# John-Ragland/pygenray

Hardware: AMD Instinct MI355X
Metric: ray-steps/sec (whole node), 1e5-ray Munk fan to 1000 km; eigenray wall-clock (higher is better)
Workload: dtype f64

## Files before the change

pygenray_amd/csrc/pgr_device.h:

```cpp
#ifndef PGR_DEVICE_H
#define PGR_DEVICE_H

struct EnvDev {
    const double2* tab;
    const double* rin;
    const double* zin;
    const double* depths;
    const double* depth_ranges;
    const double* pp;
    int nr, nz, nb;
    int row_stride;
    int z_uniform, r_uniform, b_uniform;
    int beta_zero;
    int z_pow2;
    int z_simple;
    double b_zmin, b_xlo, b_xhi;
    double z0, dz, inv_dz;
    double r0, dr, inv_dr;
    double b0, db, inv_db;
    double zlo_tol, zhi_tol, rlo_tol, rhi_tol;
    double c_lo, c_hi;
    const unsigned short* zbucket;
    int z_bucket, zb_B;
    double zb_z0, zb_inv_w;
// ... 49 lines not shown
              "kFanArgsKernargOffset together with the kernel's signature");

#define RUNNING (-1)


__device__ __forceinline__ double frcp(double b)
{
    double y = __builtin_amdgcn_rcp(b);
    double e = fma(-b, y, 1.0);
    y = fma(y, e, y);
    e = fma(-b, y, 1.0);
    y = fma(y, e, y);
    return y;
}
__device__ __forceinline__ double fdiv(double a, double b)
{
    double y = __builtin_amdgcn_rcp(b);
    double e = fma(-b, y, 1.0);
    y = fma(y, e, y);
    double q = a * y;
    double r = fma(-q, b, a);
    return fma(r, y, q);
}
__device__ __forceinline__ double frcp_seed(double b)
{
    double y = __builtin_amdgcn_rcp(b);
    double e = fma(-b, y, 1.0);
    return fma(y, e, y);
}
__device__ __forceinline__ double fdiv_y(double a, double b, double y)
{
    double q = a * y;
    double r = fma(-q, b, a);
    return fma(r, y, q);
}
__device__ __forceinline__ double frsqrt_raw(double x)
{
    double y = __builtin_amdgcn_rsq(x);
    double e = fma(-x * y, y, 1.0);
    y = fma(y * 0.5, e, y);
    e = fma(-x * y, y, 1.0);
    y = fma(y * 0.5, e, y);
    return y;
}
__device__ __forceinline__ double fsqrt(double x)
{
    double y = __builtin_amdgcn_rsq(x);
    double e = fma(-x * y, y, 1.0);
    y = fma(y * 0.5, e, y);
    double g = x * y;
    double d = fma(-g, g, x);
    double r = fma(d * 0.5, y, g);
    return (x == 0.0 || x == INFINITY) ? x : r;
}
__device__ __forceinline__ double frsqrt(double x)
{
#ifdef PGR_FMA
    return frsqrt_raw(x);
#else
    double y = __builtin_amdgcn_rsq(x);
    double e = fma(-x * y, y, 1.0);
    y = fma(y * 0.5, e, y);
    double g = x * y;
    double d = fma(-g, g, x);
    double s = fma(d * 0.5, y, g);
    y = __longlong_as_double(__double_as_longlong(y) | 1LL);
    double r = fma(-s, y, 1.0);
    double out = fma(y, r, y);
    return out;
#endif
}
__device__ __forceinline__ double pow_m02(double x, const double fifth = 0.2, const double kln2 = PGR_CR_POW_KLN2)
{
    return pgr_cr_pow_m02_k(x, fifth, kln2);
}
__device__ __forceinline__ double min_step_of(double t)
{
    long long b = __double_as_longlong(t);
    double nx = (t == 0.0) ? 4.9406564584124654e-324 : __longlong_as_double(t > 0 ? b + 1 : b - 1);
    return 10 * fabs(nx - t);
}
__device__ __forceinline__ double grid_at(double g0, double dg, int j)
{
#pragma clang fp contract(off)
    double m = (double)j * dg;
    return g0 + m;
}

__device__ __forceinline__ unsigned long long ballot64(bool b) { return __builtin_amdgcn_ballot_w64(b); }

__device__ __forceinline__ int clamp_index(int j, int hi)
{
    int r;
    asm("v_med3_i32 %0, %1, 0, %2" : "=v"(r) : "v"(j), "s"(hi));
    return r;
}

__device__ __forceinline__ int cell_uniform(double q, double g0, double dg, double inv_dg, int n)
{
    double t = (q - g0) * inv_dg;
    t = fmin(fmax(t, -1.0), (double)n);
    int j = (int)floor(t);
    double gj = grid_at(g0, dg, j), gj1 = grid_at(g0, dg, j + 1);
    j += (gj >= q) ? -1 : ((gj1 < q) ? 1 : 0);
    return min(max(j, 0), n - 2);
}

__device__ __forceinline__ int cell_search(double q, const double* __restrict__ g, int n)
{
    int lo = 0, hi = n;
    while (lo < hi) {
        int mid = (lo + hi) >> 1;
        if (g[mid] < q) lo = mid + 1; else hi = mid;
    }
    return min(max(lo - 1, 0), n - 2);
}

#define A21 (1.0 / 5)
#define A31 (3.0 / 40)
#define A32 (9.0 / 40)
#define A41 (44.0 / 45)
#define A42 (-56.0 / 15)
#define A43 (32.0 / 9)
#define A51 (19372.0 / 6561)
#define A52 (-25360.0 / 2187)
#define A53 (64448.0 / 6561)
#define A54 (-212.0 / 729)
#define A61 (9017.0 / 3168)
#define A62 (-355.0 / 33)
#define A63 (46732.0 / 5247)
#define A64 (49.0 / 176)
#define A65 (-5103.0 / 18656)
#define B1 (35.0 / 384)
#define B3 (500.0 / 1113)
#define B4 (125.0 / 192)
#define B5 (-2187.0 / 6784)
#define B6 (11.0 / 84)
#define E1 (-71.0 / 57600)
#define E3 (71.0 / 16695)
#define E4 (-71.0 / 1920)
#define E5 (17253.0 / 339200)
#define E6 (-22.0 / 525)
#define E7 (1.0 / 40)
#define C2 (1.0 / 5)
#define C3 (3.0 / 10)
#define C4 (4.0 / 5)
#define C5 (8.0 / 9)

__device__ __forceinline__ double next_up(double x)
{
    const long long b = __double_as_longlong(x);
    return __longlong_as_double((x == 0.0) ? 1LL : (b >= 0 ? b + 1 : b - 1));
}

template <bool LDS_TAB, int ZM>
struct Ctx {
    static constexpr bool ZS = (ZM == 1 || ZM == 4);
    const EnvDev& e;
    const double2* lds;
    const double* bx;
    const double* bd;
    const double* lds_z;
    const unsigned short* lds_zb;
    const double h_zb_z0, h_zb_inv_w;
    const int h_zb_B;
    const double h_zq_c0, h_zq_c1, h_zq_c2, h_zq_inv_span;
    mutable double h_zc_g0, h_zc_g1, h_zc_g2, h_zc_g3, h_zc_s0, h_zc_s1, h_zc_s2;
    mutable double r_lo, r_hi, r_yden, r_hi2;
    mutable int r_i;
    const double h_inv_dz, h_dz, h_r0, h_dr, h_inv_dr;
    const double h_zhi_tol, h_zlo_tol;
    mutable int x_guard = 0;
    mutable double zmin_eff = -INFINITY;
    const double h_b0, h_db, h_inv_db;
    const int h_nb, h_b_uniform;
    const double2* const h_tab;
    const int h_row_stride, h_z_uniform, h_z_pow2;
    const double h_z0;
    const double* const h_zin;
    const double* const h_rin;
    const int h_nz, h_nr, h_r_uniform;
    mutable double k_c2 = C2, k_c3 = C3, k_c4 = C4, k_c5 = C5, k_tiny = 1e-30, k_vert = 0.9999999998;
    __device__ __forceinline__ Ctx(const EnvDev& e_, const double2* l, const double* lz = nullptr,
                                   const unsigned short* lzb = nullptr, const double* lbx = nullptr)
        : e(e_), lds(l), bx(lbx ? lbx : e_.depth_ranges), bd(lbx ? lbx + e_.nb : e_.depths), lds_z(lz),
          lds_zb(lzb), h_zb_z0(e_.zb_z0), h_zb_inv_w(e_.zb_inv_w), h_zb_B(e_.zb_B),
          h_zq_c0(e_.zq_c0), h_zq_c1(e_.zq_c1), h_zq_c2(e_.zq_c2), h_zq_inv_span(e_.zq_inv_span),
          h_zc_g0(e_.zc_g0), h_zc_g1(e_.zc_g1), h_zc_g2(e_.zc_g2), h_zc_g3(e_.zc_g3),
          h_zc_s0(e_.zc_s0), h_zc_s1(e_.zc_s1), h_zc_s2(e_.zc_s2),
          h_inv_dz(e_.inv_dz), h_dz(e_.dz), h_r0(e_.r0), h_dr(e_.dr), h_inv_dr(e_.inv_dr),
          h_zhi_tol(e_.zhi_tol), h_zlo_tol(e_.zlo_tol), h_b0(e_.b0), h_db(e_.db),
          h_inv_db(e_.inv_db), h_nb(e_.nb), h_b_uniform(e_.b_uniform), h_tab(e_.tab),
          h_row_stride(e_.row_stride), h_z_uniform(e_.z_uniform), h_z_pow2(e_.z_pow2), h_z0(e_.z0),
          h_zin(e_.zin),
          h_rin(e_.rin), h_nz(e_.nz), h_nr(e_.nr), h_r_uniform(e_.r_uniform)
    {
        r_lo = 1.0; r_hi = 0.0; r_yden = 1.0; r_hi2 = 0.0; r_i = 0;
    }
    __device__ __forceinline__ void reset_range_cache() const
    {
        r_lo = 1.0; r_hi = 0.0; r_yden = 1.0; r_hi2 = 0.0; r_i = 0;
    }
    __device__ __forceinline__ void declare_span(double x0, double x1) const
    {
        x_guard = (x0 <= x1) && (x0 >= e.rlo_tol) && (x1 <= e.rhi_tol) && (x0 >= e.b_xlo) && (x1 <= e.b_xhi);
        zmin_eff = x_guard ? e.b_zmin : -INFINITY;
    }

    __device__ __forceinline__ int cell_z(double z, double& zj, double& zj1) const
    {
        int j;
        if (h_z_uniform) {
            j = cell_uniform(z, h_z0, h_dz, h_inv_dz, h_nz);
            zj = grid_at(h_z0, h_dz, j);
            zj1 = grid_at(h_z0, h_dz, j + 1);
        } else {
            j = cell_search(z, h_zin, h_nz);
            zj = h_zin[j];
            zj1 = h_zin[j + 1];
        }
        return j;
    }
    __device__ __forceinline__ int cell_r(double x, double& ri, double& ri1) const
    {
        int i;
        if (h_r_uniform) {
            i = cell_uniform(x, h_r0, h_dr, h_inv_dr, h_nr);
            ri = grid_at(h_r0, h_dr, i);
            ri1 = grid_at(h_r0, h_dr, i + 1);
        } else {
            i = cell_search(x, h_rin, h_nr);
            ri = h_rin[i];
            ri1 = h_rin[i + 1];
        }
        return i;
    }
    __device__ __forceinline__ void refill(double x) const
    {
        double ri, ri1;
        r_i = cell_r(x, ri, ri1);
        r_lo = ri; r_hi = ri1;
        r_yden = frcp(ri1 - ri);
        r_hi2 = (h_r_uniform && r_i + 2 <= h_nr - 1) ? grid_at(h_r0, h_dr, r_i + 2) : ri1;
    }
    __device__ __forceinline__ double weight_r(double x, int& i) const
    {
        if (!(x > r_lo && x <= r_hi)) refill(x);
        i = r_i;
        return fdiv_y(x - r_lo, r_hi - r_lo, r_yden);
    }

    __device__ __forceinline__ void lookup(double x, double z, double& c, double& cp) const
    {
        int i;
        double wx = weight_r(x, i);
        lookup_w(wx, i, z, c, cp);
    }
    struct Fetch {
        double2 v00, v01, v10, v11;
        double wy;
        double z, za, zb;
        int i, j;
    };
    __device__ __forceinline__ Fetch fetch(int i, double z) const
    {
        Fetch f;
        int j;
        if (ZM == 5) {
            const double t = fma(z, fma(z, fma(z, h_zc_g3, h_zc_g2), h_zc_g1), h_zc_g0);
            j = clamp_index((int)t, h_nz - 2);
            f.z = z; f.j = j; f.i = i;
            f.za = lds_z[j];
            f.zb = lds_z[j + 1];
            f.wy = 0.0;
            fetch_nodes(f, i, j);
            return f;
        } else if (ZM == 2 || ZM == 3) {
            int j0;
            if (ZM == 2) {
                const double t = (z - h_zb_z0) * h_zb_inv_w;
                const int k = min(max((int)floor(t), 0), h_zb_B - 1);
                j0 = lds_zb[k];
            } else {
                const double u = (z - h_zb_z0) * h_zq_inv_span;
                const double g = h_zq_c0 + u * (h_zq_c1 + u * h_zq_c2);
                j0 = min(max((int)floor(g - 0.5), 0), h_nz - 2);
            }
            const int j2 = min(j0 + 2, h_nz - 1);
            const double za = lds_z[j0], zb = lds_z[j0 + 1], zc = lds_z[j2];
            const bool up = (z > zb) & (j0 + 1 <= h_nz - 2);
            j = j0 + (up ? 1 : 0);
            const double zj = up ? zb : za, zj1 = up ? zc : zb;
            f.wy = fdiv(z - zj, zj1 - zj);
            if (LDS_TAB) {
                const double2 t0 = lds[j0], t1 = lds[j0 + 1], t2 = lds[j2];
                f.v00 = up ? t1 : t0;
                f.v01 = up ? t2 : t1;
                f.v10 = f.v00; f.v11 = f.v01;
                return f;
            }
        } else if (ZS) {
            const double t = (ZM == 4) ? z : z * h_inv_dz;
            j = clamp_index((int)t, h_nz - 2);
            f.wy = (ZM == 4) ? (z - (double)j) : (z - (double)j * h_dz) * h_inv_dz;
        } else {
            double zj, zj1;
            j = cell_z(z, zj, zj1);
            f.wy = h_z_pow2 ? (z - zj) * h_inv_dz : fdiv(z - zj, zj1 - zj);
        }
        fetch_nodes(f, i, j);
        return f;
    }
    __device__ __forceinline__ void fetch_nodes(Fetch& f, int i, int j) const
    {
        if (LDS_TAB) {
            f.v00 = lds[j];
            f.v01 = lds[j + 1];
            f.v10 = f.v00;
            f.v11 = f.v01;
        } else {
            typedef double __attribute__((ext_vector_type(2))) d2v;
            typedef const d2v __attribute__((address_space(1))) * GlobalTab;
            const GlobalTab row = (GlobalTab)h_tab + (size_t)i * h_row_stride + j;
            const d2v t00 = row[0], t01 = row[1], t10 = row[h_row_stride], t11 = row[h_row_stride + 1];
            f.v00 = make_double2(t00.x, t00.y);
            f.v01 = make_double2(t01.x, t01.y);
            f.v10 = make_double2(t10.x, t10.y);
            f.v11 = make_double2(t11.x, t11.y);
        }
    }
    __device__ __forceinline__ void blend(const Fetch& f_in, double wx, double& c, double& cp) const
    {
        Fetch f = f_in;
        if (ZM == 5) {
            if (__builtin_expect(ballot64(f.z > f.zb) != 0, 0)) {
                const bool up = (f.z > f.zb) & (f.j < h_nz - 2);
                f.j += up ? 1 : 0;
                f.za = lds_z[f.j];
                f.zb = lds_z[f.j + 1];
                fetch_nodes(f, f.i, f.j);
            }
            const double a = f.z - f.za, den = f.zb - f.za, jf = (double)f.j;
            double y = fma(jf, fma(jf, h_zc_s2, h_zc_s1), h_zc_s0);
            const double e = fma(-den, y, 1.0);
            y = fma(y, e, y);
            f.wy = fdiv_y(a, den, y);
        }
        const double wy = f.wy;
        double a = (1 - wx) * (1 - wy), b = wx * (1 - wy), cc = (1 - wx) * wy, d = wx * wy;
        c = a * f.v00.x + b * f.v10.x + cc * f.v01.x + d * f.v11.x;
        cp = a * f.v00.y + b * f.v10.y + cc * f.v01.y + d * f.v11.y;
    }
    __device__ __forceinline__ void lookup_w(double wx, int i, double z, double& c, double& cp) const
    {
        const Fetch f = fetch(i, z);
        blend(f, wx, c, cp);
    }

    __device__ __forceinline__ double bathy(double x) const
    {
        int i;
        return bathy(x, i);
    }
    __device__ __forceinline__ double bathy(double x, int& i) const
    {
        double xi, xi1;
        if (h_b_uniform) {
            i = cell_uniform(x, h_b0, h_db, h_inv_db, h_nb);
            xi = grid_at(h_b0, h_db, i);
            xi1 = grid_at(h_b0, h_db, i + 1);
        } else {
            i = cell_search(x, bx, h_nb);
            xi = bx[i];
            xi1 = bx[i + 1];
        }
        double w = fdiv(x - xi, xi1 - xi);
        return (1 - w) * bd[i] + w * bd[i + 1];
    }

    __device__ __forceinline__ void rhs(double x, double z, double pz, double& d0, double& d1,
                                        double& d2, double& c) const
    {
        int i;
        double wx = weight_r(x, i);
        rhs_w(wx, i, z, pz, d0, d1, d2, c);
    }
    __device__ __forceinline__ void rhs_w(double wx, int i, double z, double pz, double& d0, double& d1,
                                          double& d2, double& c) const
    {
        rhs_f(fetch(i, z), wx, pz, d0, d1, d2, c);
    }
    __device__ __forceinline__ void rhs_f(const Fetch& ft, double wx, double pz, double& d0, double& d1,
                                          double& d2, double& c) const
    {
        double cp;
        blend(ft, wx, c, cp);
        double arg = 1.0 - (c * c) * (pz * pz);
        arg = fmax(arg, k_tiny);
        double fact = frsqrt(arg);
        double rc = frcp_seed(c);
        d0 = fdiv_y(fact, c, rc);
        d1 = c * pz * fact;
        d2 = fdiv_y(-fact * cp, c * c, rc * rc);
    }

    __device__ __forceinline__ void step_weights(double t, double h, double (&w)[5], int (&ic)[5]) const
    {
        const double xs[5] = {t + k_c2 * h, t + k_c3 * h, t + k_c4 * h, t + k_c5 * h, t + 1.0 * h};
        if (__builtin_expect((t >= r_lo) & (xs[4] <= r_hi), 1)) {
            const double den = r_hi - r_lo;
#pragma unroll
            for (int s = 0; s < 5; s++) {
                w[s] = fdiv_y(xs[s] - r_lo, den, r_yden);
                ic[s] = r_i;
            }
        } else {
            if (h_r_uniform && (t > r_hi) && (t <= r_hi2) && (r_hi2 > r_hi)) {
                r_lo = r_hi; r_hi = r_hi2; r_i++;
                r_yden = frcp(r_hi - r_lo);
                r_hi2 = (r_i + 2 <= h_nr - 1) ? grid_at(h_r0, h_dr, r_i + 2) : r_hi;
            }
            if (h_r_uniform && (t >= r_lo) && (t <= r_hi) && (xs[4] <= r_hi2)) {
                const double a_den = r_hi - r_lo, b_den = r_hi2 - r_hi;
                const double b_yden = frcp(b_den);
#pragma unroll
                for (int s = 0; s < 5; s++) {
                    const bool in_b = xs[s] > r_hi;
                    const double lo = in_b ? r_hi : r_lo, den = in_b ? b_den : a_den, yd = in_b ? b_yden : r_yden;
                    w[s] = fdiv_y(xs[s] - lo, den, yd);
                    ic[s] = r_i + (in_b ? 1 : 0);
                }
            } else {
#pragma unroll
                for (int s = 0; s < 5; s++) w[s] = weight_r(xs[s], ic[s]);
            }
        }
    }

    __device__ __forceinline__ unsigned events(double x, double z, double pz, double c) const
    {
        double pc = pz * c;
        unsigned g = ((z < 0) & (pc < 0) & (pc >= -1.0)) ? 1u : 0u;
        bool above = (z < zmin_eff);
        if (__builtin_expect(!x_guard, 0)) above = (z < e.b_zmin) & (x >= e.b_xlo) & (x <= e.b_xhi);
        const bool near_bottom = (pc > 0) & (pc <= 1.0) & !above;
        const bool near_vertical = (fabs(pc) > k_vert) & (fabs(pc) <= 1.0);
        if (near_bottom | near_vertical) {
            if (near_bottom) {
                if (z > bathy(x)) g |= 2u;
            }
            if (near_vertical) {
                double th = pgr_cr_asin(pc) * (180.0 / M_PI);
                if (fabs(th) > (90 - 1e-3)) g |= 4u;
            }
        }
        bool outside = (z > h_zhi_tol) | (z < h_zlo_tol);
        if (__builtin_expect(!x_guard, 0)) outside |= (x < e.rlo_tol) | (x > e.rhi_tol);
        if (outside) g |= 8u;
        return g;
    }
};

__device__ __forceinline__ double rms3(double a, double b, double c, double sqrt3 = 1.7320508075688772,
                                       double inv_sqrt3 = 0.57735026918962584)
{
    return fdiv_y(fsqrt(a * a + b * b + c * c), sqrt3, inv_sqrt3);
}

struct Dense {
    double h;
    double q[3][4];
    __device__ __forceinline__ void eval(double t_old, double y0, double y1, double y2, double t,
                                         double& o0, double& o1, double& o2) const
    {
        double x = fdiv(t - t_old, h);
        double p1 = x, p2 = p1 * x, p3 = p2 * x, p4 = p3 * x;
        o0 = h * (q[0][0] * p1 + q[0][1] * p2 + q[0][2] * p3 + q[0][3] * p4) + y0;
        o1 = h * (q[1][0] * p1 + q[1][1] * p2 + q[1][2] * p3 + q[1][3] * p4) + y1;
        o2 = h * (q[2][0] * p1 + q[2][1] * p2 + q[2][2] * p3 + q[2][3] * p4) + y2;
    }
};

#define PQ(k1, k3, k4, k5, k6, k7, j)                                                   \
    ((k1) * P1##j + (k3) * P3##j + (k4) * P4##j + (k5) * P5##j + (k6) * P6##j + (k7) * P7##j)
#define P10 1.0
#define P11 (-8048581381.0 / 2820520608)
#define P12 (8663915743.0 / 2820520608)
#define P13 (-12715105075.0 / 11282082432)
#define P30 0.0
#define P31 (131558114200.0 / 32700410799)
#define P32 (-68118460800.0 / 10900136933)
#define P33 (87487479700.0 / 32700410799)
#define P40 0.0
#define P41 (-1754552775.0 / 470086768)
#define P42 (14199869525.0 / 1410260304)
#define P43 (-10690763975.0 / 1880347072)
#define P50 0.0
#define P51 (127303824393.0 / 49829197408)
#define P52 (-318862633887.0 / 49829197408)
#define P53 (701980252875.0 / 199316789632)
#define P60 0.0
#define P61 (-282668133.0 / 205662961)
#define P62 (2019193451.0 / 616988883)
#define P63 (-1453857185.0 / 822651844)
#define P70 0.0
#define P71 (40617522.0 / 29380423)
#define P72 (-110615467.0 / 29380423)
#define P73 (69997945.0 / 29380423)

#define PGR_FORM_Q()                                                                    \
    do {                                                                                \
        D.h = h;                                                                        \
        D.q[0][0] = f0;                                                                 \
        D.q[0][1] = PQ(f0, k30, k40, k50, k60, k70, 1);                                 \
        D.q[0][2] = PQ(f0, k30, k40, k50, k60, k70, 2);                                 \
        D.q[0][3] = PQ(f0, k30, k40, k50, k60, k70, 3);                                 \
        D.q[1][0] = f1;                                                                 \
        D.q[1][1] = PQ(f1, k31, k41, k51, k61, k71, 1);                                 \
        D.q[1][2] = PQ(f1, k31, k41, k51, k61, k71, 2);                                 \
        D.q[1][3] = PQ(f1, k31, k41, k51, k61, k71, 3);                                 \
        D.q[2][0] = f2;                                                                 \
        D.q[2][1] = PQ(f2, k32, k42, k52, k62, k72, 1);                                 \
        D.q[2][2] = PQ(f2, k32, k42, k52, k62, k72, 2);                                 \
        D.q[2][3] = PQ(f2, k32, k42, k52, k62, k72, 3);                                 \
    } while (0)

#define PGR_SB() __builtin_amdgcn_sched_barrier(0)
#if defined(PGR_TIMING) || defined(PGR_SVC_TIMING)
#define PGR_STAMP_(k)                                                                                 \
    do {                                                                                             \
        unsigned long long _t;                                                                       \
        PGR_SB();                                                                                    \
        asm volatile("s_waitcnt lgkmcnt(0)\n\ts_memtime %0\n\ts_waitcnt lgkmcnt(0)" : "=s"(_t) : : "memory"); \
        tacc[k] += (unsigned)_t - tprev;                                                             \
        tprev = (unsigned)_t;                                                                        \
        PGR_SB();                                                                                    \
    } while (0)
#endif
#ifdef PGR_TIMING
#define PGR_STAMP(k) PGR_STAMP_(k)
#else
#define PGR_STAMP(k) do { } while (0)
#endif
#ifdef PGR_SVC_TIMING
#define PGR_SSTAMP(k) PGR_STAMP_(k)
#else
#define PGR_SSTAMP(k) do { } while (0)
#endif
#define PGR_KEEP2(a_, b_) do { if (ZM == 5) asm volatile("" : "+v"(a_), "+v"(b_)); } while (0)
#define PGR_KEEP6(a_, b_, c_, d_, e_, f_) do { if (ZM == 5) asm volatile("" : "+v"(a_), "+v"(b_), "+v"(c_), "+v"(d_), "+v"(e_), "+v"(f_)); } while (0)
#define PGR_RK_STAGES(T_, H_)                                                                        \
    double k30, k31, k32, k40, k41, k42, k50, k51, k52, k60, k61, k62, k70, k71, k72;                \
    PGR_RK_STAGES_BODY(T_, H_)
#define PGR_RK_STAGES_BODY(T_, H_)                                                                   \
    double k20, k21, k22, cs;                                                                        \
    double wr[5];                                                                                    \
    int ir[5];                                                                                       \
    PGR_STAMP(1);                                                                                    \
    C.step_weights(T_, H_, wr, ir);                                                                  \
    PGR_STAMP(2);                                                                                    \
                           \
    const double zs2 = y1 + (f1 * vA21) * (H_), ps2 = y2 + (f2 * vA21) * (H_);                         \
    PGR_STAMP(3);                                                                                    \
    const auto ft2 = C.fetch(ir[0], zs2);                                                            \
    PGR_SB();                                                                                        \
    double a31 = f1 * vA31, a32 = f2 * vA31, a41 = f1 * vA41, a42 = f2 * vA41, a51 = f1 * vA51,           \
           a52 = f2 * vA51, a61 = f1 * vA61, a62 = f2 * vA61;                                           \
    double bs0 = f0 * vB1, bs1 = f1 * vB1, bs2 = f2 * vB1, es0 = f0 * vE1, es1 = f1 * vE1, es2 = f2 * vE1; \
    PGR_KEEP6(a31, a32, a41, a42, a51, a52); PGR_KEEP2(a61, a62);                                    \
    PGR_KEEP6(bs0, bs1, bs2, es0, es1, es2);                                                         \
    PGR_SB();                                                                                        \
    C.rhs_f(ft2, wr[0], ps2, k20, k21, k22, cs);                                                     \
    PGR_STAMP(4);                                                                                    \
    a31 = a31 + k21 * vA32; a32 = a32 + k22 * vA32;                                                    \
    const double zs3 = y1 + a31 * (H_), ps3 = y2 + a32 * (H_);                                       \
    PGR_STAMP(5);                                                                                    \
    const auto ft3 = C.fetch(ir[1], zs3);                                                            \
    PGR_SB();                                                                                        \
    a41 = a41 + k21 * vA42; a42 = a42 + k22 * vA42;                                                    \
    a51 = a51 + k21 * vA52; a52 = a52 + k22 * vA52;                                                    \
    a61 = a61 + k21 * vA62; a62 = a62 + k22 * vA62;                                                    \
    PGR_KEEP6(a41, a42, a51, a52, a61, a62);                                                         \
    PGR_SB();                                                                                        \
    C.rhs_f(ft3, wr[1], ps3, k30, k31, k32, cs);                                                     \
    PGR_STAMP(6);                                                                                    \
    a41 = a41 + k31 * vA43; a42 = a42 + k32 * vA43;                                                    \
    const double zs4 = y1 + a41 * (H_), ps4 = y2 + a42 * (H_);                                       \
    PGR_STAMP(7);                                                                                    \
    const auto ft4 = C.fetch(ir[2], zs4);                                                            \
    PGR_SB();                                                                                        \
    a51 = a51 + k31 * vA53; a52 = a52 + k32 * vA53;                                                    \
    a61 = a61 + k31 * vA63; a62 = a62 + k32 * vA63;                                                    \
    bs0 = bs0 + k30 * vB3; bs1 = bs1 + k31 * vB3; bs2 = bs2 + k32 * vB3;                                \
    es0 = es0 + k30 * vE3; es1 = es1 + k31 * vE3; es2 = es2 + k32 * vE3;                                \
    PGR_KEEP6(bs0, bs1, bs2, es0, es1, es2); PGR_KEEP2(a51, a52); PGR_KEEP2(a61, a62);               \
    PGR_SB();                                                                                        \
    C.rhs_f(ft4, wr[2], ps4, k40, k41, k42, cs);                                                     \
    PGR_STAMP(8);                                                                                    \
    a51 = a51 + k41 * vA54; a52 = a52 + k42 * vA54;                                                    \
    const double zs5 = y1 + a51 * (H_), ps5 = y2 + a52 * (H_);                                       \
    PGR_STAMP(9);                                                                                    \
    const auto ft5 = C.fetch(ir[3], zs5);                                                            \
    PGR_SB();                                                                                        \
    a61 = a61 + k41 * vA64; a62 = a62 + k42 * vA64;                                                    \
    bs0 = bs0 + k40 * vB4; bs1 = bs1 + k41 * vB4; bs2 = bs2 + k42 * vB4;                                \
    es0 = es0 + k40 * vE4; es1 = es1 + k41 * vE4; es2 = es2 + k42 * vE4;                                \
    PGR_KEEP6(bs0, bs1, bs2, es0, es1, es2); PGR_KEEP2(a61, a62);                                    \
    PGR_SB();                                                                                        \
    C.rhs_f(ft5, wr[3], ps5, k50, k51, k52, cs);                                                     \
    PGR_STAMP(10);                                                                                   \
    a61 = a61 + k51 * vA65; a62 = a62 + k52 * vA65;                                                    \
    const double zs6 = y1 + a61 * (H_), ps6 = y2 + a62 * (H_);                                       \
    PGR_STAMP(11);                                                                                   \
    const auto ft6 = C.fetch(ir[4], zs6);                                                            \
    PGR_SB();                                                                                        \
    bs0 = bs0 + k50 * vB5; bs1 = bs1 + k51 * vB5; bs2 = bs2 + k52 * vB5;                                \
    es0 = es0 + k50 * vE5; es1 = es1 + k51 * vE5; es2 = es2 + k52 * vE5;                                \
    PGR_KEEP6(bs0, bs1, bs2, es0, es1, es2);                                                         \
    PGR_SB();                                                                                        \
    C.rhs_f(ft6, wr[4], ps6, k60, k61, k62, cs);                                                     \
    PGR_STAMP(12);                                                                                   \
                                                    \
    bs1 = bs1 + k61 * vB6; bs2 = bs2 + k62 * vB6;                                                      \
    const double n1 = y1 + (H_) * bs1, n2 = y2 + (H_) * bs2;                                         \
                                                           \
    PGR_STAMP(13);                                                                                   \
    const auto ft7 = C.fetch(ir[4], n1);                                                             \
    PGR_SB();                                                                                        \
    bs0 = bs0 + k60 * vB6;                                                                            \
    const double n0 = y0 + (H_) * bs0;                                                               \
    es0 = es0 + k60 * vE6; es1 = es1 + k61 * vE6; es2 = es2 + k62 * vE6;                                \
    { double n0k_ = n0; PGR_KEEP2(n0k_, es0); PGR_KEEP2(es1, es2); }                                 \
    PGR_SB();                                                                                        \
    double c_new;                                                                                    \
    C.rhs_f(ft7, wr[4], n2, k70, k71, k72, c_new);                                                   \
    PGR_STAMP(14);                                                                                   \
                                               \
    es0 = es0 + k70 * vE7; es1 = es1 + k71 * vE7; es2 = es2 + k72 * vE7

struct SaveGrid {
    const double* r;
    double x0, x1, step;
    int S, formula;
    __device__ __forceinline__ double at(int j) const
    {
        if (formula) return (j >= S - 1) ? x1 : grid_at(x0, step, j);
        return r[j];
    }
    __device__ __forceinline__ int nearest(double t, double inv_step) const
    {
        double g = (t - x0) * inv_step;
        g = fmin(fmax(g, 0.0), (double)(S - 1));
        int j = (int)rint(g);
        int best = max(j - 1, 0);
        double bd = fabs(at(best) - t);
        for (int k = best + 1; k <= min(j + 1, S - 1); k++) {
            double d = fabs(at(k) - t);
            if (d < bd) { bd = d; best = k; }
        }
        return best;
    }
};

#endif
```

pygenray_amd/csrc/pgr_fan_kernel.h:

```cpp
#ifndef PGR_FAN_KERNEL_H
#define PGR_FAN_KERNEL_H

template <bool LDS_TAB, int ZM, int SAVE, bool PERSIST, bool LOG = false>
__global__ void __launch_bounds__(512)
pgr_fan_kernel(const EnvDev* __restrict__ env_p, typename FanKernelArgs<LOG>::type a)
{
    const EnvDev& env = *env_p;
    extern __shared__ double2 lds_tab[];
    double* const lds_after_tab = (double*)(lds_tab + (LDS_TAB ? env.nz : 0));
    double* const lds_z = lds_after_tab;
    unsigned short* const lds_zb = (unsigned short*)(lds_z + env.nz);
    if (LDS_TAB) {
        for (int j = threadIdx.x; j < env.nz; j += blockDim.x) lds_tab[j] = env.tab[j];
    }
    if (ZM == 2 || ZM == 3 || ZM == 5) {
        for (int j = threadIdx.x; j < env.nz; j += blockDim.x) lds_z[j] = env.zin[j];
        if (ZM == 2) for (int j = threadIdx.x; j < env.zb_B; j += blockDim.x) lds_zb[j] = env.zbucket[j];
    }
    double* const lds_bx = (a.bathy_lds_off >= 0) ? (double*)((char*)lds_tab + a.bathy_lds_off) : nullptr;
    if (lds_bx) {
        for (int j = threadIdx.x; j < env.nb; j += blockDim.x) {
            lds_bx[j] = env.depth_ranges[j];
            lds_bx[env.nb + j] = env.depths[j];
        }
// ... 59 lines not shown

    double t = a.x0, y0 = 0, y1 = 0, y2 = 0;
    if (valid) {
        y0 = q_y0[3 * ray + 0];
        y1 = q_y0[3 * ray + 1];
        y2 = q_y0[3 * ray + 2];
    }
    double f0 = 0, f1 = 0, f2 = 0, h_abs = 0;
    unsigned g = 0;
    int status = valid ? RUNNING : PGR_RAY_OK;
    if (valid && (q_flags & PGR_SKIP_NAN_Y0) && (y2 != y2)) status = PGR_RAY_SKIPPED;
    bool need_init = true, rejected = false, parked = false;
    int nb = 0, ns = 0, n_steps = 0, n_rej = 0;
    int jnext = 0;
    double rnext = 0;
    double pk_tnew = 0;
    unsigned pk_active = 0;
    int waited = 0;
    int trips = 0, services = 0, fallbacks = 0;
    const double min_step_bound = 10 * 0x1p-52 * fmax(fabs(a.x0), fabs(a.x1)) + 1e-300;
    const int max_steps32 = (int)(a.max_steps < 0x7fffffff ? a.max_steps : 0x7fffffff);
    const int guard_limit = (max_steps32 < attempt_limit ? max_steps32 : attempt_limit);
#if defined(PGR_TIMING) || defined(PGR_SVC_TIMING)
    unsigned tacc[24];
    for (int k = 0; k < 24; k++) tacc[k] = 0;
    unsigned tprev = (unsigned)clock64();
#endif
    const int64_t out_off = ray * q_stride_ray;
#define Tp (a.T + out_off)
#define Zp (a.Z + out_off)
#define Pp (a.P + out_off)
    constexpr bool BLK = (SAVE == 3);
    static_assert(!(BLK && LDS_TAB), "the blocked sample layout is instantiated for the HBM-table kernels only");
    double* const blk = (double*)((char*)lds_tab + (BLK ? a.blk_lds_off : 0)) + (wv * 768 + (int)(threadIdx.x & 63));
    auto blk_flush = [&](int jb) __attribute__((always_inline)) {
        const int64_t o = ((int64_t)jb * a.N + ray) * 4;
        typedef double d2 __attribute__((ext_vector_type(2)));
        const d2 t0 = {blk[0], blk[64]}, t1 = {blk[128], blk[192]};
        const d2 z0 = {blk[256], blk[320]}, z1 = {blk[384], blk[448]};
        const d2 p0 = {blk[512], blk[576]}, p1 = {blk[640], blk[704]};
        __builtin_nontemporal_store(t0, (d2*)(a.T + o)); __builtin_nontemporal_store(t1, (d2*)(a.T + o + 2));
        __builtin_nontemporal_store(z0, (d2*)(a.Z + o)); __builtin_nontemporal_store(z1, (d2*)(a.Z + o + 2));
        __builtin_nontemporal_store(p0, (d2*)(a.P + o)); __builtin_nontemporal_store(p1, (d2*)(a.P + o + 2));
    };
    auto emit_sample = [&](int j, double vt, double vz, double vp) __attribute__((always_inline)) {
        if (BLK) {
            double* const e = blk + (j & 3) * 64;
            e[0] = vt; e[256] = vz; e[512] = vp;
            if ((j & 3) == 3) blk_flush(j >> 2);
            return;
        }
        const int64_t o = (int64_t)j * a.stride_smp;
        if (LDS_TAB) { Tp[o] = vt; Zp[o] = vz; Pp[o] = vp; }
        else {
            __builtin_nontemporal_store(vt, &Tp[o]);
            __builtin_nontemporal_store(vz, &Zp[o]);
            __builtin_nontemporal_store(vp, &Pp[o]);
        }
    };

#define PGR_VCONST(n) double v##n = n; asm volatile("" : "+v"(v##n))
    PGR_VCONST(A21);
    PGR_VCONST(A31);
    PGR_VCONST(A32);
    PGR_VCONST(A41);
    PGR_VCONST(A42);
    PGR_VCONST(A43);
    PGR_VCONST(A51);
    PGR_VCONST(A52);
    PGR_VCONST(A53);
    PGR_VCONST(A54);
    PGR_VCONST(A61);
    PGR_VCONST(A62);
    PGR_VCONST(A63);
    PGR_VCONST(A64);
    PGR_VCONST(A65);
    PGR_VCONST(B1);
    PGR_VCONST(B3);
    PGR_VCONST(B4);
    PGR_VCONST(B5);
    PGR_VCONST(B6);
    PGR_VCONST(E1);
    PGR_VCONST(E3);
    PGR_VCONST(E4);
    PGR_VCONST(E5);
    PGR_VCONST(E6);
    PGR_VCONST(E7);
#undef PGR_VCONST
    constexpr bool PIN_P = (SAVE != 0 && ZM != 0 && ZM != 3);
#define PGR_VCONST_IF(c, n) double v##n = n; if (c) asm volatile("" : "+v"(v##n))
    PGR_VCONST_IF(PIN_P, P11);
    PGR_VCONST_IF(PIN_P, P12);
    PGR_VCONST_IF(PIN_P, P13);
    PGR_VCONST_IF(PIN_P, P31);
    PGR_VCONST_IF(PIN_P, P32);
    PGR_VCONST_IF(PIN_P, P33);
    PGR_VCONST_IF(PIN_P, P41);
    PGR_VCONST_IF(PIN_P, P42);
    PGR_VCONST_IF(PIN_P, P43);
    PGR_VCONST_IF(PIN_P, P51);
    PGR_VCONST_IF(PIN_P, P52);
    PGR_VCONST_IF(PIN_P, P53);
    PGR_VCONST_IF(PIN_P, P61);
    PGR_VCONST_IF(PIN_P, P62);
    PGR_VCONST_IF(PIN_P, P63);
    PGR_VCONST_IF(PIN_P, P71);
    PGR_VCONST_IF(PIN_P, P72);
    PGR_VCONST_IF(PIN_P, P73);
#undef PGR_VCONST_IF
    constexpr bool PIN_LITERALS = (SAVE == 0 || ZM == 3);
    if (PIN_LITERALS) {
#define PGR_PIN(x) asm volatile("" : "+v"(x))
        PGR_PIN(C.k_c2); PGR_PIN(C.k_c3); PGR_PIN(C.k_c4); PGR_PIN(C.k_c5); PGR_PIN(C.k_tiny); PGR_PIN(C.k_vert);
        PGR_PIN(SAFETY); PGR_PIN(MIN_FACTOR); PGR_PIN(MAX_FACTOR);
        PGR_PIN(SQRT3); PGR_PIN(INV_SQRT3);
        PGR_PIN(POW_FIFTH); PGR_PIN(POW_KLN2);
#undef PGR_PIN
    }
    constexpr int PIN_ZC = (SAVE != 0 ? 2 : 1);
    if (ZM == 5 && PIN_ZC >= 1) {
        asm volatile("" : "+v"(C.h_zc_g2));
        asm volatile("" : "+v"(C.h_zc_s1));
    }
    if (ZM == 5 && PIN_ZC >= 2) {
        asm volatile("" : "+v"(C.h_zc_g0));
        asm volatile("" : "+v"(C.h_zc_g1));
        asm volatile("" : "+v"(C.h_zc_g3));
        asm volatile("" : "+v"(C.h_zc_s0));
        asm volatile("" : "+v"(C.h_zc_s2));
    }
    constexpr bool KEEPK = !(ZM == 5 && SAVE != 0);
    double k30 = 0, k31 = 0, k32 = 0, k40 = 0, k41 = 0, k42 = 0, k50 = 0, k51 = 0, k52 = 0, k60 = 0, k61 = 0, k62 = 0,
           k70 = 0, k71 = 0, k72 = 0;
    do {
        bool run, pend;
        unsigned long long pm;
        do {
        trips++;
        PGR_STAMP(0);
        if (status == RUNNING && !parked && !need_init) {
            bool too_small = false;
            if (__builtin_expect(ballot64(h_abs < min_step_bound) != 0, 0)) {
                double min_step = min_step_of(t);
                if (!rejected && h_abs < min_step) h_abs = min_step;
                too_small = h_abs < min_step;
                if (too_small) status = PGR_RAY_STEP_TOO_SMALL;
            }
            double h = h_abs;
            double t_new = t + h;
            if ((t_new - t_bound) > 0) t_new = t_bound;
            h = t_new - t;
            h_abs = fabs(h);

            PGR_RK_STAGES_BODY(t, h);
            double sc0 = atol + fmax(fabs(y0), fabs(n0)) * rtol;
            double sc1 = atol + fmax(fabs(y1), fabs(n1)) * rtol;
            double sc2 = atol + fmax(fabs(y2), fabs(n2)) * rtol;
            double er0 = fdiv(es0 * h, sc0);
            double er1 = fdiv(es1 * h, sc1);
            double er2 = fdiv(es2 * h, sc2);
            double error_norm = rms3(er0, er1, er2, SQRT3, INV_SQRT3);
            PGR_STAMP(15);

            const bool accepted = !too_small && (error_norm < 1);
            const bool reject = !too_small && !accepted;
            const double pw = SAFETY * pow_m02(error_norm, POW_FIFTH, POW_KLN2);
            double fac_acc = (pw < MAX_FACTOR) ? pw : MAX_FACTOR;
            fac_acc = (rejected && !(fac_acc < 1)) ? 1.0 : fac_acc;
            const double fac_rej = (pw > MIN_FACTOR) ? pw : MIN_FACTOR;
            h_abs = h_abs * (accepted ? fac_acc : fac_rej);
            rejected = reject;
            n_rej += reject ? 1 : 0;
            const bool guards_due = trips > guard_limit;
            if (__builtin_expect(guards_due, 0)) {
                const bool over = (n_rej + n_steps) > attempt_limit;
                status = (reject & over) ? PGR_RAY_MAX_STEPS : status;
                trips = trips < 0x7f000000 ? trips : 0x7f000000;
            }
            PGR_STAMP(16);

            if (accepted) {
                n_steps++;
                unsigned g_new = C.events(t_new, n1, n2, c_new);
                PGR_STAMP(17);
                unsigned up = (~g) & g_new, down = g & (~g_new);
                unsigned active = (up & 3u) | ((up | down) & 12u);
                g = g_new;
                bool want_samples = save && (jnext < S - 1) && (rnext <= t_new);
                const bool scipy_order = exact_samples || (rnext < t);
                Dense D;
                if (active) {
                    parked = true;
                    pk_active = active;
                    pk_tnew = t_new;
                } else {
                    if (want_samples) {
                        if (scipy_order) {
                            PGR_FORM_Q();
                            while (jnext < S - 1 && rnext <= t_new) {
                                double o0, o1, o2;
                                D.eval(t, y0, y1, y2, rnext, o0, o1, o2);
                                emit_sample(jnext, o0, SGN(o1), SGN(o2));
                                jnext++;
                                rnext = G.at(jnext);
                            }
                        } else {
                            const double inv_h = frcp_seed(h);
#define PGR_KSUM(k1, k3, k4, k5, k6, k7)                                                          \
    __builtin_fma(k1, b1, __builtin_fma(k3, b3, __builtin_fma(k4, b4, __builtin_fma(k5, b5,      \
                  __builtin_fma(k6, b6, (k7) * b7)))))
#define PGR_SAMPLE_LOOP(NEXT)                                                                     \
    while (jnext < S - 1 && rnext <= t_new) {                                                     \
        const double xi = (rnext - t) * inv_h, x2 = xi * xi;                                      \
        const double b1 = xi * __builtin_fma(xi, __builtin_fma(xi, __builtin_fma(xi, vP13, vP12), vP11), P10); \
        const double b3 = x2 * __builtin_fma(xi, __builtin_fma(xi, vP33, vP32), vP31);               \
        const double b4 = x2 * __builtin_fma(xi, __builtin_fma(xi, vP43, vP42), vP41);               \
        const double b5 = x2 * __builtin_fma(xi, __builtin_fma(xi, vP53, vP52), vP51);               \
        const double b6 = x2 * __builtin_fma(xi, __builtin_fma(xi, vP63, vP62), vP61);               \
        const double b7 = x2 * __builtin_fma(xi, __builtin_fma(xi, vP73, vP72), vP71);               \
        emit_sample(jnext, __builtin_fma(h, PGR_KSUM(f0, k30, k40, k50, k60, k70), y0),            \
                    SGN(__builtin_fma(h, PGR_KSUM(f1, k31, k41, k51, k61, k71), y1)),               \
                    SGN(__builtin_fma(h, PGR_KSUM(f2, k32, k42, k52, k62, k72), y2)));              \
        jnext++;                                                                                  \
        rnext = NEXT;                                                                             \
    }
                            if (SAVE == 1 || SAVE == 3 || G.formula) { PGR_SAMPLE_LOOP(grid_at(G.x0, G.step, jnext)) }
                            else { PGR_SAMPLE_LOOP(G.r[jnext]) }
#undef PGR_SAMPLE_LOOP
#undef PGR_KSUM
                        }
                    }
                    t = t_new; y0 = n0; y1 = n1; y2 = n2;
                    f0 = k70; f1 = k71; f2 = k72;
                    status = ((t - t_bound) >= 0) ? PGR_RAY_OK : status;
                    if (__builtin_expect(guards_due, 0))
                        status = (status == RUNNING && n_steps > max_steps32) ? PGR_RAY_MAX_STEPS : status;
                }
                PGR_STAMP(18);
            }
        }
        PGR_STAMP(19);
        run = (status == RUNNING);
        pend = run && (parked || need_init);
        pm = ballot64(pend);
        } while (pm == 0 && ballot64(run) != 0);
        asm volatile("" : "+s"(pm));
        if (pm) {
            waited++;
            const bool nobody_steps = ballot64(run && !pend) == 0;
            if (__popcll(pm) >= a.park_lanes || waited > a.park_trips || nobody_steps) {
                waited = 0;
                services++;
                PGR_SSTAMP(23);
                typedef const EnvDev __attribute__((address_space(4))) EnvConst;
                EnvConst* es_p = (EnvConst*)env_p;
                asm volatile("" : "+s"(es_p));
                EnvConst& es = *es_p;
                const char __attribute__((address_space(4))) * ks_p =
                    (const char __attribute__((address_space(4))) *)__builtin_amdgcn_kernarg_segment_ptr();
                asm volatile("" : "+s"(ks_p));
                const FanArgs __attribute__((address_space(4))) & as = *(const FanArgs __attribute__((address_space(4))) *)(ks_p + kFanArgsKernargOffset);
                constexpr bool SVC_BATCH = LDS_TAB && ZM == 4;
                double svc_c_lo = es.c_lo, svc_c_hi = es.c_hi;
                double svc_rlo_tol = 0, svc_rhi_tol = 0, svc_b_xlo = 0, svc_b_xhi = 0, svc_inv_dsave = 0;
                int svc_beta_zero = 0;
                uint32_t svc_flags = 0;
                if (SVC_BATCH) {
                    svc_rlo_tol = es.rlo_tol; svc_rhi_tol = es.rhi_tol;
                    svc_b_xlo = es.b_xlo; svc_b_xhi = es.b_xhi;
                    svc_beta_zero = es.beta_zero;
                    svc_flags = as.flags;
                    if (save) svc_inv_dsave = as.inv_dsave;
                }
#define PGR_SVC(batched_, lazy_) (SVC_BATCH ? (batched_) : (lazy_))
                if (pend && parked) {
                    parked = false;
                    const unsigned active = pk_active;
                    const double t_new = pk_tnew, h = t_new - t;
                    Dense D;
                    PGR_SSTAMP(0);
                    if (KEEPK) {
                        PGR_FORM_Q();
                    } else {
                        PGR_RK_STAGES(t, h);
                        (void)n0; (void)c_new; (void)es0; (void)es1; (void)es2;
                        PGR_FORM_Q();
                    }
                    if (SVC_BATCH)
                        asm volatile("" : "+s"(svc_c_lo), "+s"(svc_c_hi), "+s"(svc_rlo_tol), "+s"(svc_rhi_tol), "+s"(svc_b_xlo),
                                          "+s"(svc_b_xhi), "+s"(svc_beta_zero), "+s"(svc_flags));
                    PGR_SSTAMP(1);
                    int ev = -1;
                    double best = 0;
                    const bool with_bbox = (active == 9u);
                    const unsigned act = with_bbox ? 1u : active;
                    if ((a.flags & PGR_EXACT_BISECTION) == 0 && (act == 1u || act == 2u)) {
                        const bool bottom = (act == 2u);
                        const double q0 = D.q[1][0], q1 = D.q[1][1], q2 = D.q[1][2], q3 = D.q[1][3];
                        double bs = 0, be = 0;
                        int cell_s = 0, cell_e = 0;
                        if (bottom) { bs = C.bathy(t, cell_s); be = C.bathy(t_new, cell_e); }
                        double zb = y1 + h * (q0 + q1 + q2 + q3);
                        double Fa = bottom ? (y1 - bs) : y1;
                        double Fb = bottom ? (zb - be) : zb;
                        bool pre = bottom ? (Fa <= 0 && Fb > 0) : (Fa >= 0 && Fb < 0);
                        double xa = t, xb = t_new;
                        bool live = false;
                        const bool any_bottom = ballot64(bottom) != 0;
                        const bool chord = ballot64(bottom && cell_s != cell_e) == 0;
                        PGR_SSTAMP(2);
                        if (pre) {
                            const double bslope = bottom ? (be - bs) : 0.0;
                            double lo = 0.0, hi = 1.0;
// ... 379 lines not shown
```

Baseline: 26.48 billion.

## Split RK stage RHS so its tail overlaps the next stage's global fetch

For the global-table path (non-LDS), each RK stage's right-hand side is split in two. The part that feeds the next stage's depth address (c, fact, d1) runs first, and the cp blend, reciprocal and divisions are deferred until after the next stage's table fetch has been issued. The aim is to hide global-memory latency behind the division work. The error-scale reciprocals are also moved into the shadow of the last fetch. The cost is more live registers, which may lower occupancy.

New measurement: 26.47 billion. Within noise of the previous version (-0.1%).

```diff
diff --git a/pygenray_amd/csrc/pgr_device.h b/pygenray_amd/csrc/pgr_device.h
--- a/pygenray_amd/csrc/pgr_device.h
+++ b/pygenray_amd/csrc/pgr_device.h
@@ -225,6 +225,14 @@
     const long long b = __double_as_longlong(x);
     return __longlong_as_double((x == 0.0) ? 1LL : (b >= 0 ? b + 1 : b - 1));
 }
+
+struct BlendRest {
+    double a, b, cc, d, y00, y10, y01, y11;
+};
+struct RhsRest {
+    BlendRest bl;
+    double fact;
+};
 
 template <bool LDS_TAB, int ZM>
 struct Ctx {
@@ -402,9 +410,8 @@
             f.v11 = make_double2(t11.x, t11.y);
         }
     }
-    __device__ __forceinline__ void blend(const Fetch& f_in, double wx, double& c, double& cp) const
-    {
-        Fetch f = f_in;
+    __device__ __forceinline__ void settle_cell(Fetch& f) const
+    {
         if (ZM == 5) {
             if (__builtin_expect(ballot64(f.z > f.zb) != 0, 0)) {
                 const bool up = (f.z > f.zb) & (f.j < h_nz - 2);
@@ -419,6 +426,24 @@
             y = fma(y, e, y);
             f.wy = fdiv_y(a, den, y);
         }
+    }
+    __device__ __forceinline__ void blend_c(const Fetch& f_in, double wx, double& c, BlendRest& r) const
+    {
+        Fetch f = f_in;
+        settle_cell(f);
+        const double wy = f.wy;
+        r.a = (1 - wx) * (1 - wy); r.b = wx * (1 - wy); r.cc = (1 - wx) * wy; r.d = wx * wy;
+        c = r.a * f.v00.x + r.b * f.v10.x + r.cc * f.v01.x + r.d * f.v11.x;
+        r.y00 = f.v00.y; r.y10 = f.v10.y; r.y01 = f.v01.y; r.y11 = f.v11.y;
+    }
+    __device__ __forceinline__ void blend_cp(const BlendRest& r, double& cp) const
+    {
+        cp = r.a * r.y00 + r.b * r.y10 + r.cc * r.y01 + r.d * r.y11;
+    }
+    __device__ __forceinline__ void blend(const Fetch& f_in, double wx, double& c, double& cp) const
+    {
+        Fetch f = f_in;
+        settle_cell(f);
         const double wy = f.wy;
         double a = (1 - wx) * (1 - wy), b = wx * (1 - wy), cc = (1 - wx) * wy, d = wx * wy;
         c = a * f.v00.x + b * f.v10.x + cc * f.v01.x + d * f.v11.x;
@@ -475,6 +500,23 @@
         d0 = fdiv_y(fact, c, rc);
         d1 = c * pz * fact;
         d2 = fdiv_y(-fact * cp, c * c, rc * rc);
+    }
+    static constexpr bool SPLIT_RHS = !LDS_TAB;
+    __device__ __forceinline__ void rhs_addr(const Fetch& ft, double wx, double pz, double& d1, double& c, RhsRest& r) const
+    {
+        blend_c(ft, wx, c, r.bl);
+        double arg = 1.0 - (c * c) * (pz * pz);
+        arg = fmax(arg, k_tiny);
+        r.fact = frsqrt(arg);
+        d1 = c * pz * r.fact;
+    }
+    __device__ __forceinline__ void rhs_rest(const RhsRest& r, double c, double& d0, double& d2) const
+    {
+        double cp;
+        blend_cp(r.bl, cp);
+        double rc = frcp_seed(c);
+        d0 = fdiv_y(r.fact, c, rc);
+        d2 = fdiv_y(-r.fact * cp, c * c, rc * rc);
     }
 
     __device__ __forceinline__ void step_weights(double t, double h, double (&w)[5], int (&ic)[5]) const
@@ -620,90 +662,120 @@
 #else
 #define PGR_SSTAMP(k) do { } while (0)
 #endif
+#define PGR_KEEP1(a_) do { if (ZM == 5) asm volatile("" : "+v"(a_)); } while (0)
 #define PGR_KEEP2(a_, b_) do { if (ZM == 5) asm volatile("" : "+v"(a_), "+v"(b_)); } while (0)
 #define PGR_KEEP6(a_, b_, c_, d_, e_, f_) do { if (ZM == 5) asm volatile("" : "+v"(a_), "+v"(b_), "+v"(c_), "+v"(d_), "+v"(e_), "+v"(f_)); } while (0)
 #define PGR_RK_STAGES(T_, H_)                                                                        \
     double k30, k31, k32, k40, k41, k42, k50, k51, k52, k60, k61, k62, k70, k71, k72;                \
     PGR_RK_STAGES_BODY(T_, H_)
-#define PGR_RK_STAGES_BODY(T_, H_)                                                                   \
+#define PGR_RK_STAGES_BODY(T_, H_) PGR_RK_STAGES_BODY_X(T_, H_, (void)0)
+#define PGR_RK_STAGES_BODY_X(T_, H_, SHADOW7_)                                                       \
     double k20, k21, k22, cs;                                                                        \
     double wr[5];                                                                                    \
     int ir[5];                                                                                       \
+    RhsRest rr;                                                                                      \
     PGR_STAMP(1);                                                                                    \
     C.step_weights(T_, H_, wr, ir);                                                                  \
     PGR_STAMP(2);                                                                                    \
-                           \
-    const double zs2 = y1 + (f1 * vA21) * (H_), ps2 = y2 + (f2 * vA21) * (H_);                         \
+                \
+    const double zs2 = y1 + (f1 * vA21) * (H_);                                                      \
+    double ps2 = y2 + (f2 * vA21) * (H_);                                                            \
     PGR_STAMP(3);                                                                                    \
     const auto ft2 = C.fetch(ir[0], zs2);                                                            \
     PGR_SB();                                                                                        \
-    double a31 = f1 * vA31, a32 = f2 * vA31, a41 = f1 * vA41, a42 = f2 * vA41, a51 = f1 * vA51,           \
-           a52 = f2 * vA51, a61 = f1 * vA61, a62 = f2 * vA61;                                           \
-    double bs0 = f0 * vB1, bs1 = f1 * vB1, bs2 = f2 * vB1, es0 = f0 * vE1, es1 = f1 * vE1, es2 = f2 * vE1; \
+    double a31 = f1 * vA31, a32 = f2 * vA31, a41 = f1 * vA41, a42 = f2 * vA41, a51 = f1 * vA51,      \
+           a52 = f2 * vA51, a61 = f1 * vA61, a62 = f2 * vA61;                                        \
+    double bs0 = f0 * vB1, bs1 = f1 * vB1, bs2 = f2 * vB1, es0 = f0 * vE1, es1 = f1 * vE1, es2 = f2 * vE1;\
     PGR_KEEP6(a31, a32, a41, a42, a51, a52); PGR_KEEP2(a61, a62);                                    \
     PGR_KEEP6(bs0, bs1, bs2, es0, es1, es2);                                                         \
     PGR_SB();                                                                                        \
-    C.rhs_f(ft2, wr[0], ps2, k20, k21, k22, cs);                                                     \
+    if (C.SPLIT_RHS) C.rhs_addr(ft2, wr[0], ps2, k21, cs, rr);                                       \
+    else C.rhs_f(ft2, wr[0], ps2, k20, k21, k22, cs);                                                \
     PGR_STAMP(4);                                                                                    \
-    a31 = a31 + k21 * vA32; a32 = a32 + k22 * vA32;                                                    \
-    const double zs3 = y1 + a31 * (H_), ps3 = y2 + a32 * (H_);                                       \
+    a31 = a31 + k21 * vA32;                                                                          \
+    if (!C.SPLIT_RHS) a32 = a32 + k22 * vA32;                                                        \
+    const double zs3 = y1 + a31 * (H_);                                                              \
+    double ps3;                                                                                      \
+    if (!C.SPLIT_RHS) ps3 = y2 + a32 * (H_);                                                         \
     PGR_STAMP(5);                                                                                    \
     const auto ft3 = C.fetch(ir[1], zs3);                                                            \
     PGR_SB();                                                                                        \
-    a41 = a41 + k21 * vA42; a42 = a42 + k22 * vA42;                                                    \
-    a51 = a51 + k21 * vA52; a52 = a52 + k22 * vA52;                                                    \
-    a61 = a61 + k21 * vA62; a62 = a62 + k22 * vA62;                                                    \
-    PGR_KEEP6(a41, a42, a51, a52, a61, a62);                                                         \
-    PGR_SB();                                                                                        \
-    C.rhs_f(ft3, wr[1], ps3, k30, k31, k32, cs);                                                     \
+    if (C.SPLIT_RHS) { C.rhs_rest(rr, cs, k20, k22); a32 = a32 + k22 * vA32; ps3 = y2 + a32 * (H_); }\
+    a41 = a41 + k21 * vA42; a42 = a42 + k22 * vA42;                                                  \
+    a51 = a51 + k21 * vA52; a52 = a52 + k22 * vA52;                                                  \
+    a61 = a61 + k21 * vA62; a62 = a62 + k22 * vA62;                                                  \
+    PGR_KEEP6(a41, a42, a51, a52, a61, a62); if (C.SPLIT_RHS) PGR_KEEP1(ps3);                        \
+    PGR_SB();                                                                                        \
+    if (C.SPLIT_RHS) C.rhs_addr(ft3, wr[1], ps3, k31, cs, rr);                                       \
+    else C.rhs_f(ft3, wr[1], ps3, k30, k31, k32, cs);                                                \
     PGR_STAMP(6);                                                                                    \
-    a41 = a41 + k31 * vA43; a42 = a42 + k32 * vA43;                                                    \
-    const double zs4 = y1 + a41 * (H_), ps4 = y2 + a42 * (H_);                                       \
+    a41 = a41 + k31 * vA43;                                                                          \
+    if (!C.SPLIT_RHS) a42 = a42 + k32 * vA43;                                                        \
+    const double zs4 = y1 + a41 * (H_);                                                              \
+    double ps4;                                                                                      \
+    if (!C.SPLIT_RHS) ps4 = y2 + a42 * (H_);                                                         \
     PGR_STAMP(7);                                                                                    \
     const auto ft4 = C.fetch(ir[2], zs4);                                                            \
     PGR_SB();                                                                                        \
-    a51 = a51 + k31 * vA53; a52 = a52 + k32 * vA53;                                                    \
-    a61 = a61 + k31 * vA63; a62 = a62 + k32 * vA63;                                                    \
-    bs0 = bs0 + k30 * vB3; bs1 = bs1 + k31 * vB3; bs2 = bs2 + k32 * vB3;                                \
-    es0 = es0 + k30 * vE3; es1 = es1 + k31 * vE3; es2 = es2 + k32 * vE3;                                \
-    PGR_KEEP6(bs0, bs1, bs2, es0, es1, es2); PGR_KEEP2(a51, a52); PGR_KEEP2(a61, a62);               \
-    PGR_SB();                                                                                        \
-    C.rhs_f(ft4, wr[2], ps4, k40, k41, k42, cs);                                                     \
+    if (C.SPLIT_RHS) { C.rhs_rest(rr, cs, k30, k32); a42 = a42 + k32 * vA43; ps4 = y2 + a42 * (H_); }\
+    a51 = a51 + k31 * vA53; a52 = a52 + k32 * vA53;                                                  \
+    a61 = a61 + k31 * vA63; a62 = a62 + k32 * vA63;                                                  \
+    bs0 = bs0 + k30 * vB3; bs1 = bs1 + k31 * vB3; bs2 = bs2 + k32 * vB3;                             \
+    es0 = es0 + k30 * vE3; es1 = es1 + k31 * vE3; es2 = es2 + k32 * vE3;                             \
+    PGR_KEEP6(bs0, bs1, bs2, es0, es1, es2); PGR_KEEP2(a51, a52); PGR_KEEP2(a61, a62); if (C.SPLIT_RHS) PGR_KEEP1(ps4);\
+    PGR_SB();                                                                                        \
+    if (C.SPLIT_RHS) C.rhs_addr(ft4, wr[2], ps4, k41, cs, rr);                                       \
+    else C.rhs_f(ft4, wr[2], ps4, k40, k41, k42, cs);                                                \
     PGR_STAMP(8);                                                                                    \
-    a51 = a51 + k41 * vA54; a52 = a52 + k42 * vA54;                                                    \
-    const double zs5 = y1 + a51 * (H_), ps5 = y2 + a52 * (H_);                                       \
+    a51 = a51 + k41 * vA54;                                                                          \
+    if (!C.SPLIT_RHS) a52 = a52 + k42 * vA54;                                                        \
+    const double zs5 = y1 + a51 * (H_);                                                              \
+    double ps5;                                                                                      \
+    if (!C.SPLIT_RHS) ps5 = y2 + a52 * (H_);                                                         \
     PGR_STAMP(9);                                                                                    \
     const auto ft5 = C.fetch(ir[3], zs5);                                                            \
     PGR_SB();                                                                                        \
-    a61 = a61 + k41 * vA64; a62 = a62 + k42 * vA64;                                                    \
-    bs0 = bs0 + k40 * vB4; bs1 = bs1 + k41 * vB4; bs2 = bs2 + k42 * vB4;                                \
-    es0 = es0 + k40 * vE4; es1 = es1 + k41 * vE4; es2 = es2 + k42 * vE4;                                \
-    PGR_KEEP6(bs0, bs1, bs2, es0, es1, es2); PGR_KEEP2(a61, a62);                                    \
-    PGR_SB();                                                                                        \
-    C.rhs_f(ft5, wr[3], ps5, k50, k51, k52, cs);                                                     \
+    if (C.SPLIT_RHS) { C.rhs_rest(rr, cs, k40, k42); a52 = a52 + k42 * vA54; ps5 = y2 + a52 * (H_); }\
+    a61 = a61 + k41 * vA64; a62 = a62 + k42 * vA64;                                                  \
+    bs0 = bs0 + k40 * vB4; bs1 = bs1 + k41 * vB4; bs2 = bs2 + k42 * vB4;                             \
+    es0 = es0 + k40 * vE4; es1 = es1 + k41 * vE4; es2 = es2 + k42 * vE4;                             \
+    PGR_KEEP6(bs0, bs1, bs2, es0, es1, es2); PGR_KEEP2(a61, a62); if (C.SPLIT_RHS) PGR_KEEP1(ps5);   \
+    PGR_SB();                                                                                        \
+    if (C.SPLIT_RHS) C.rhs_addr(ft5, wr[3], ps5, k51, cs, rr);                                       \
+    else C.rhs_f(ft5, wr[3], ps5, k50, k51, k52, cs);                                                \
     PGR_STAMP(10);                                                                                   \
-    a61 = a61 + k51 * vA65; a62 = a62 + k52 * vA65;                                                    \
-    const double zs6 = y1 + a61 * (H_), ps6 = y2 + a62 * (H_);                                       \
+    a61 = a61 + k51 * vA65;                                                                          \
+    if (!C.SPLIT_RHS) a62 = a62 + k52 * vA65;                                                        \
+    const double zs6 = y1 + a61 * (H_);                                                              \
+    double ps6;                                                                                      \
+    if (!C.SPLIT_RHS) ps6 = y2 + a62 * (H_);                                                         \
     PGR_STAMP(11);                                                                                   \
     const auto ft6 = C.fetch(ir[4], zs6);                                                            \
     PGR_SB();                                                                                        \
-    bs0 = bs0 + k50 * vB5; bs1 = bs1 + k51 * vB5; bs2 = bs2 + k52 * vB5;                                \
-    es0 = es0 + k50 * vE5; es1 = es1 + k51 * vE5; es2 = es2 + k52 * vE5;                                \
-    PGR_KEEP6(bs0, bs1, bs2, es0, es1, es2);                                                         \
-    PGR_SB();                                                                                        \
-    C.rhs_f(ft6, wr[4], ps6, k60, k61, k62, cs);                                                     \
+    if (C.SPLIT_RHS) { C.rhs_rest(rr, cs, k50, k52); a62 = a62 + k52 * vA65; ps6 = y2 + a62 * (H_); }\
+    bs0 = bs0 + k50 * vB5; bs1 = bs1 + k51 * vB5; bs2 = bs2 + k52 * vB5;                             \
+    es0 = es0 + k50 * vE5; es1 = es1 + k51 * vE5; es2 = es2 + k52 * vE5;                             \
+    PGR_KEEP6(bs0, bs1, bs2, es0, es1, es2); if (C.SPLIT_RHS) PGR_KEEP1(ps6);                        \
+    PGR_SB();                                                                                        \
+    if (C.SPLIT_RHS) C.rhs_addr(ft6, wr[4], ps6, k61, cs, rr);                                       \
+    else C.rhs_f(ft6, wr[4], ps6, k60, k61, k62, cs);                                                \
     PGR_STAMP(12);                                                                                   \
                                                     \
-    bs1 = bs1 + k61 * vB6; bs2 = bs2 + k62 * vB6;                                                      \
-    const double n1 = y1 + (H_) * bs1, n2 = y2 + (H_) * bs2;                                         \
+    bs1 = bs1 + k61 * vB6;                                                                           \
+    if (!C.SPLIT_RHS) bs2 = bs2 + k62 * vB6;                                                         \
+    const double n1 = y1 + (H_) * bs1;                                                               \
+    double n2;                                                                                       \
+    if (!C.SPLIT_RHS) n2 = y2 + (H_) * bs2;                                                          \
                                                            \
     PGR_STAMP(13);                                                                                   \
     const auto ft7 = C.fetch(ir[4], n1);                                                             \
     PGR_SB();                                                                                        \
-    bs0 = bs0 + k60 * vB6;                                                                            \
+    if (C.SPLIT_RHS) { C.rhs_rest(rr, cs, k60, k62); bs2 = bs2 + k62 * vB6; n2 = y2 + (H_) * bs2; }  \
+    bs0 = bs0 + k60 * vB6;                                                                           \
     const double n0 = y0 + (H_) * bs0;                                                               \
-    es0 = es0 + k60 * vE6; es1 = es1 + k61 * vE6; es2 = es2 + k62 * vE6;                                \
-    { double n0k_ = n0; PGR_KEEP2(n0k_, es0); PGR_KEEP2(es1, es2); }                                 \
+    es0 = es0 + k60 * vE6; es1 = es1 + k61 * vE6; es2 = es2 + k62 * vE6;                             \
+    if (C.SPLIT_RHS) { SHADOW7_; }                                                                   \
+    { double n0k_ = n0; PGR_KEEP2(n0k_, es0); PGR_KEEP2(es1, es2); if (C.SPLIT_RHS) PGR_KEEP1(n2); } \
     PGR_SB();                                                                                        \
     double c_new;                                                                                    \
     C.rhs_f(ft7, wr[4], n2, k70, k71, k72, c_new);                                                   \
diff --git a/pygenray_amd/csrc/pgr_fan_kernel.h b/pygenray_amd/csrc/pgr_fan_kernel.h
--- a/pygenray_amd/csrc/pgr_fan_kernel.h
+++ b/pygenray_amd/csrc/pgr_fan_kernel.h
@@ -235,13 +235,24 @@
             h = t_new - t;
             h_abs = fabs(h);
 
-            PGR_RK_STAGES_BODY(t, h);
-            double sc0 = atol + fmax(fabs(y0), fabs(n0)) * rtol;
-            double sc1 = atol + fmax(fabs(y1), fabs(n1)) * rtol;
-            double sc2 = atol + fmax(fabs(y2), fabs(n2)) * rtol;
-            double er0 = fdiv(es0 * h, sc0);
-            double er1 = fdiv(es1 * h, sc1);
-            double er2 = fdiv(es2 * h, sc2);
+            double sc0, sc1, sc2, rs0, rs1, rs2, er0, er1, er2;
+#define PGR_ERR_SCALES                                                                               \
+    sc0 = atol + fmax(fabs(y0), fabs(n0)) * rtol;                                                    \
+    sc1 = atol + fmax(fabs(y1), fabs(n1)) * rtol;                                                    \
+    sc2 = atol + fmax(fabs(y2), fabs(n2)) * rtol
+            PGR_RK_STAGES_BODY_X(t, h, PGR_ERR_SCALES; rs0 = frcp_seed(sc0); rs1 = frcp_seed(sc1); rs2 = frcp_seed(sc2);
+                                 PGR_KEEP6(sc0, sc1, sc2, rs0, rs1, rs2));
+            if (C.SPLIT_RHS) {
+                er0 = fdiv_y(es0 * h, sc0, rs0);
+                er1 = fdiv_y(es1 * h, sc1, rs1);
+                er2 = fdiv_y(es2 * h, sc2, rs2);
+            } else {
+                PGR_ERR_SCALES;
+                er0 = fdiv(es0 * h, sc0);
+                er1 = fdiv(es1 * h, sc1);
+                er2 = fdiv(es2 * h, sc2);
+            }
+#undef PGR_ERR_SCALES
             double error_norm = rms3(er0, er1, er2, SQRT3, INV_SQRT3);
             PGR_STAMP(15);
 
```
